# OpenRobotLab/EmbodiedScan

Hardware: NVIDIA H100
Metric: training scans/sec mv-3ddet 20-view (ResNet-50/16 + MinkResNet34, 480x640, 100k pts) (higher is better)
Workload: dtype bf16

## Files before the change

embodiedscan_b200/csrc/scratch.cu:

```cuda
#include <mutex>

#include "common.cuh"

namespace {

__global__ void sum_partial_rows_kernel(const float* __restrict__ part, int n_parts, long long width, float* __restrict__ out,
                                        int accumulate) {
  const long long j = blockIdx.x * (long long)blockDim.x + threadIdx.x;
  if (j >= width) return;
  float s = accumulate ? out[j] : 0.f;
  for (int p = 0; p < n_parts; ++p) s += part[(long long)p * width + j];
  out[j] = s;
}

}

int esb_sm_count() {
  static int sms[64] = {};
  int dev = 0;
  cudaGetDevice(&dev);
  if (dev >= 64) return 132;
  if (sms[dev] == 0) {
    int n = 132;
    cudaDeviceGetAttribute(&n, cudaDevAttrMultiProcessorCount, dev);
    sms[dev] = n;
  }
  return sms[dev];
}

namespace {
constexpr unsigned long long kScratchKeepBytes = 512ull << 20;
std::mutex g_pool_mutex;
cudaMemPool_t g_pool[64] = {};

cudaMemPool_t scratch_pool(int dev, cudaStream_t s) {
  if (dev < 0 || dev >= 64) return nullptr;
  std::lock_guard<std::mutex> lock(g_pool_mutex);
  if (g_pool[dev] == nullptr) {
    cudaStreamCaptureStatus st = cudaStreamCaptureStatusNone;
    cudaStreamIsCapturing(s, &st);
    if (st != cudaStreamCaptureStatusNone) return nullptr;
    cudaMemPoolProps props = {};
    props.allocType = cudaMemAllocationTypePinned;
    props.location.type = cudaMemLocationTypeDevice;
    props.location.id = dev;
    cudaMemPool_t pool = nullptr;
    if (cudaMemPoolCreate(&pool, &props) != cudaSuccess) return nullptr;
    unsigned long long keep = kScratchKeepBytes;
    cudaMemPoolSetAttribute(pool, cudaMemPoolAttrReleaseThreshold, &keep);
    g_pool[dev] = pool;
  }
  return g_pool[dev];
}
}

cudaError_t esb_scratch_alloc(void** p, size_t bytes, cudaStream_t s) {
  int dev = 0;
  cudaGetDevice(&dev);
  const size_t n = bytes > 0 ? bytes : 16;
  cudaMemPool_t pool = scratch_pool(dev, s);
  return pool != nullptr ? cudaMallocFromPoolAsync(p, n, pool, s) : cudaMallocAsync(p, n, s);
}

cudaError_t esb_scratch_free(void* p, cudaStream_t s) { return cudaFreeAsync(p, s); }

int esb_sum_partial_rows(const float* part, int n_parts, long long width, float* out, int accumulate, cudaStream_t s) {
  if (width == 0) return ESB_OK;
  sum_partial_rows_kernel<<<esb_div_up(width, 256), 256, 0, s>>>(part, n_parts, width, out, accumulate);
  ESB_CUDA_LAUNCH_CHECK("sum_partial_rows_kernel");
  return ESB_OK;
}
```

embodiedscan_b200/csrc/spconv_tc.cu:

```cuda
#include "tc_common.cuh"

using namespace esb_tc;

namespace {

__global__ void tile_mask_kernel(const int* __restrict__ nbr, int K, int n, uint32_t* __restrict__ masks) {
  const int tile = blockIdx.x, r = threadIdx.x;
  const int row = tile * TC_M + r;
  uint32_t m = 0;
  if (row < n)
    for (int k = 0; k < K; ++k)
      if (nbr[(long long)k * n + row] >= 0) m |= 1u << k;
  m = __reduce_or_sync(0xffffffffu, m);
  __shared__ uint32_t s[4];
  if ((r & 31) == 0) s[r >> 5] = m;
  __syncthreads();
  if (r == 0) masks[tile] = s[0] | s[1] | s[2] | s[3];
}

template <int N_TILE, int STAGES, bool B_MN>
__global__ void __launch_bounds__(384, 1)
spconv_tc_fwd_kernel(const __nv_bfloat16* __restrict__ x, const __grid_constant__ CUtensorMap tmw,
                     const int* __restrict__ nbr, const uint32_t* __restrict__ masks, __nv_bfloat16* __restrict__ y,
                     int n_out, int cin, int cout, int K) {
  constexpr int A_BYTES = A_STAGE_BYTES;
  constexpr int B_STAGE_BYTES = N_TILE * 128;
  constexpr int STAGE_BYTES = A_BYTES + B_STAGE_BYTES;
  constexpr int LAG = STAGES - 2;
  constexpr int NPROD = 128;
  constexpr int NCONS = 256;
  constexpr int PITCH = N_TILE + 4;
  static_assert(TC_M * PITCH * 4 <= STAGES * STAGE_BYTES, "the accumulator image reuses the stage buffers");
  extern __shared__ __align__(1024) uint8_t smem_raw[];
  uint8_t* smem = (uint8_t*)(((uintptr_t)smem_raw + 1023) & ~(uintptr_t)1023);
  uint64_t* full_bar = (uint64_t*)(smem + STAGES * STAGE_BYTES);
  uint64_t* empty_bar = full_bar + STAGES;
  uint64_t* accum_bar = empty_bar + STAGES;
  float* img = reinterpret_cast<float*>(smem);
  __shared__ int idx_s[2][NPROD];

  const int tile = blockIdx.x;
  const int n0 = blockIdx.y * N_TILE;
  const uint32_t mask = masks[tile];
  const int nchunk = cin / TC_BK;
  const int total = __popc(mask) * nchunk;

  if (threadIdx.x == 0) {
    for (int s = 0; s < STAGES; ++s) {
      mbar_init(&full_bar[s], NPROD + 1);
      mbar_init(&empty_bar[s], NCONS / 32);
    }
    mbar_init(accum_bar, NCONS);
    asm volatile("fence.mbarrier_init.release.cluster;" ::: "memory");
    tma_prefetch_desc(&tmw);
  }
  __syncthreads();

  if (threadIdx.x >= NCONS) {
    const int t = threadIdx.x - NCONS;
    const int sub = t & 7, rgrp = t >> 3;
    const uint32_t sw = (uint32_t)(rgrp & 7);
    const uint32_t a_thread_off = (uint32_t)((rgrp >> 3) * 1024 + (rgrp & 7) * 128) + ((sub ^ sw) << 4);
    int it = 0, kcount = 0;
    const int my_row = tile * TC_M + t;
    int v_next = (mask && my_row < n_out) ? nbr[(long long)(__ffs(mask) - 1) * n_out + my_row] : -1;
    for (uint32_t mk = mask; mk; mk &= mk - 1, ++kcount) {
      const int k = __ffs(mk) - 1;
      int* idx_buf = idx_s[kcount & 1];
      idx_buf[t] = v_next;
      asm volatile("bar.sync 1, %0;" ::"n"(NPROD) : "memory");
      {
        const uint32_t rest = mk & (mk - 1);
        v_next = (rest && my_row < n_out) ? nbr[(long long)(__ffs(rest) - 1) * n_out + my_row] : -1;
      }
      int src[8];
#pragma unroll
      for (int i = 0; i < 8; ++i) src[i] = idx_buf[rgrp + 16 * i];
      for (int c = 0; c < nchunk; ++c, ++it) {
        const int s = it % STAGES;
        if (it >= STAGES) mbar_wait(&empty_bar[s], ((it / STAGES) - 1) & 1);
        const uint32_t stage_base = smem_u32(smem + s * STAGE_BYTES);
        if (t == 0) {
          mbar_expect_tx(&full_bar[s], B_STAGE_BYTES);
          const uint32_t b_base = stage_base + A_BYTES;
          if (B_MN) {
#pragma unroll
            for (int a = 0; a < N_TILE / 64; ++a) tma_load_2d(&tmw, &full_bar[s], b_base + a * 8192, n0 + a * 64, k * cin + c * TC_BK);
          } else {
            tma_load_2d(&tmw, &full_bar[s], b_base, c * TC_BK, k * cout + n0);
          }
        }
        const uint32_t a_base = stage_base + a_thread_off;
#pragma unroll
        for (int i = 0; i < 8; ++i)
          cp_async16_ca(a_base + i * 2048, x + (long long)(src[i] >= 0 ? src[i] : 0) * cin + c * TC_BK + sub * 8,
                        src[i] >= 0 ? 16 : 0);
        cp_async_commit();
        if (it >= LAG) {
          cp_async_wait<LAG>();
          fence_proxy_async();
          mbar_arrive(&full_bar[(it - LAG) % STAGES]);
        }
      }
    }
    cp_async_wait<0>();
    fence_proxy_async();
    for (int d = (total > LAG ? total - LAG : 0); d < total; ++d) mbar_arrive(&full_bar[d % STAGES]);

    const int row = tile * TC_M + t;
    if (total > 0) mbar_wait(accum_bar, 0);
    __nv_bfloat16* yrow = y + (long long)row * cout + n0;
#pragma unroll 1
    for (int c0 = 0; c0 < N_TILE; c0 += 32) {
      uint32_t v[32];
      if (total > 0) {
        img_ld<32>(img, PITCH, t, c0, v);
      } else {
#pragma unroll
        for (int i = 0; i < 32; ++i) v[i] = 0u;
      }
      if (row < n_out) {
#pragma unroll
        for (int q = 0; q < 4; ++q) {
          uint4 o;
          o.x = pack_bf16(v[8 * q + 0], v[8 * q + 1]);
          o.y = pack_bf16(v[8 * q + 2], v[8 * q + 3]);
          o.z = pack_bf16(v[8 * q + 4], v[8 * q + 5]);
          o.w = pack_bf16(v[8 * q + 6], v[8 * q + 7]);
          *reinterpret_cast<uint4*>(yrow + c0 + 8 * q) = o;
        }
      }
    }
  } else if (total > 0) {
    const int wg = threadIdx.x >> 7;
    float acc[N_TILE / 2];
    for (int it = 0; it < total; ++it) {
      const int s = it % STAGES;
      mbar_wait(&full_bar[s], (it / STAGES) & 1);
      const uint32_t a_addr = smem_u32(smem + s * STAGE_BYTES) + wg * 8192;
      const uint32_t b_addr = smem_u32(smem + s * STAGE_BYTES) + A_BYTES;
      wgmma_fence();
#pragma unroll
      for (int kk = 0; kk < TC_BK / 16; ++kk) {
        const uint64_t bd = B_MN ? make_desc(b_addr + kk * 2048, 8192, 1024) : make_desc(b_addr + kk * 32, 16, 1024);
        wgmma_bf16<N_TILE, 0, B_MN ? 1 : 0>(acc, make_desc(a_addr + kk * 32, 16, 1024), bd, it > 0 || kk > 0);
      }
      wgmma_commit();
      wgmma_wait<1>();
      if (it > 0 && (threadIdx.x & 31) == 0) mbar_arrive(&empty_bar[(it - 1) % STAGES]);
    }
    wgmma_wait<0>();
    acc_fence<N_TILE / 2>(acc);
    asm volatile("bar.sync 2, %0;" ::"n"(NCONS) : "memory");
    acc_store<N_TILE>(acc, img, PITCH, wg * 64, threadIdx.x & 127);
    mbar_arrive(accum_bar);
  }
}

template <int N_TILE, int STAGES>
__global__ void __launch_bounds__(384, 1)
spconv_tc_wgrad_kernel(const __nv_bfloat16* __restrict__ x, const __nv_bfloat16* __restrict__ dy,
                       const int* __restrict__ pair_in, const int* __restrict__ pair_out,
                       const int* __restrict__ k_offsets, float* __restrict__ part, int cin, int cout, int K,
                       int chunk_pairs) {
  constexpr int A_BYTES = 64 * 256;
  constexpr int B_BYTES = 64 * N_TILE * 2;
  constexpr int STAGE_BYTES = A_BYTES + B_BYTES;
  constexpr int LAG = STAGES - 2;
  constexpr int NCONS = 256;
  constexpr int PITCH = N_TILE + 4;
  static_assert(128 * PITCH * 4 <= STAGES * STAGE_BYTES, "the accumulator image reuses the stage buffers");
  extern __shared__ __align__(1024) uint8_t smem_raw[];
  uint8_t* smem = (uint8_t*)(((uintptr_t)smem_raw + 1023) & ~(uintptr_t)1023);
  uint64_t* full_bar = (uint64_t*)(smem + STAGES * STAGE_BYTES);
  uint64_t* empty_bar = full_bar + STAGES;
  uint64_t* accum_bar = empty_bar + STAGES;

  int k = 0, chunk = blockIdx.x, p_beg = 0, p_end = 0;
  for (; k < K; ++k) {
    p_beg = k_offsets[k];
    p_end = k_offsets[k + 1];
    const int nch = (p_end - p_beg + chunk_pairs - 1) / chunk_pairs;
    if (chunk < nch) break;
    chunk -= nch;
  }
  if (k >= K) return;
  const int ci0 = blockIdx.y * 128, co0 = blockIdx.z * N_TILE;
  const int s_beg = p_beg + chunk * chunk_pairs;
  const int s_end = min(p_end, s_beg + chunk_pairs);
  const int total = (s_end - s_beg + 63) / 64;

  if (threadIdx.x == 0) {
    for (int s = 0; s < STAGES; ++s) {
      mbar_init(&full_bar[s], 128);
      mbar_init(&empty_bar[s], NCONS / 32);
    }
    mbar_init(accum_bar, NCONS);
    asm volatile("fence.mbarrier_init.release.cluster;" ::: "memory");
  }
  __syncthreads();
  const int a_ch = min(128, cin - ci0);

  if (threadIdx.x >= NCONS) {
    const int t = threadIdx.x - NCONS;
    const int warp = t >> 5;
    const int mc = t & 15, kk0 = t >> 4;
    const bool a_ok_ch = mc * 8 < a_ch;
    int ri[8], ro[8];
#pragma unroll
    for (int q = 0; q < 8; ++q) {
      const int p = s_beg + kk0 + 8 * q;
      ri[q] = p < s_end ? pair_in[p] : -1;
      ro[q] = p < s_end ? pair_out[p] : -1;
    }
    for (int it = 0; it < total; ++it) {
      const int s = it % STAGES;
      if (it >= STAGES) mbar_wait(&empty_bar[s], ((it / STAGES) - 1) & 1);
      const uint32_t a_base = smem_u32(smem + s * STAGE_BYTES);
      const uint32_t b_base = a_base + A_BYTES;
#pragma unroll
      for (int q = 0; q < 8; ++q) {
        const int kk = kk0 + 8 * q;
        const bool ok = ri[q] >= 0 && a_ok_ch;
        const uint32_t dst = a_base + (mc >> 3) * 8192 + (kk >> 3) * 1024 + (kk & 7) * 128 + (((mc & 7) ^ (kk & 7)) << 4);
        cp_async16_cg(dst, x + (long long)(ok ? ri[q] : 0) * cin + ci0 + mc * 8, ok ? 16 : 0);
      }
#pragma unroll
      for (int q = 0; q < N_TILE / 16; ++q) {
        const int idx = q * 128 + t;
        const int kk = idx / (N_TILE / 8), nc = idx % (N_TILE / 8);
        int rr;
        if (N_TILE == 128) {
          rr = ro[q];
        } else {
          const int p = s_beg + it * 64 + kk;
          rr = p < s_end ? pair_out[p] : -1;
        }
        const uint32_t dst = b_base + (nc >> 3) * 8192 + (kk >> 3) * 1024 + (kk & 7) * 128 + (((nc & 7) ^ (kk & 7)) << 4);
        cp_async16_cg(dst, dy + (long long)(rr >= 0 ? rr : 0) * cout + co0 + nc * 8, rr >= 0 ? 16 : 0);
      }
      cp_async_commit();
      if (it + 1 < total) {
#pragma unroll
        for (int q = 0; q < 8; ++q) {
          const int p = s_beg + (it + 1) * 64 + kk0 + 8 * q;
          ri[q] = p < s_end ? pair_in[p] : -1;
          ro[q] = p < s_end ? pair_out[p] : -1;
        }
      }
      if (it >= LAG) {
        cp_async_wait<LAG>();
        fence_proxy_async();
        mbar_arrive(&full_bar[(it - LAG) % STAGES]);
      }
    }
    cp_async_wait<0>();
    fence_proxy_async();
    for (int d = (total > LAG ? total - LAG : 0); d < total; ++d) mbar_arrive(&full_bar[d % STAGES]);

    mbar_wait(accum_bar, 0);
    const float* stg = reinterpret_cast<const float*>(smem);
    const int lane = t & 31;
    for (int rr = 0; rr < 32; ++rr) {
      const int r = warp * 32 + rr;
      const int ci = ci0 + r;
      if (ci >= cin) break;
      float* dwrow = part + ((long long)blockIdx.x * cin + ci) * cout + co0;
#pragma unroll
      for (int c = lane * 4; c < N_TILE; c += 128)
        *reinterpret_cast<float4*>(dwrow + c) = *reinterpret_cast<const float4*>(stg + r * PITCH + c);
    }
  } else {
    const int wg = threadIdx.x >> 7;
    float acc[N_TILE / 2];
    for (int it = 0; it < total; ++it) {
      const int s = it % STAGES;
      mbar_wait(&full_bar[s], (it / STAGES) & 1);
      const uint32_t a_addr = smem_u32(smem + s * STAGE_BYTES) + wg * 8192;
      const uint32_t b_addr = smem_u32(smem + s * STAGE_BYTES) + A_BYTES;
      wgmma_fence();
#pragma unroll
      for (int kk = 0; kk < 4; ++kk)
        wgmma_bf16<N_TILE, 1, 1>(acc, make_desc(a_addr + kk * 2048, 8192, 1024), make_desc(b_addr + kk * 2048, 8192, 1024), it > 0 || kk > 0);
      wgmma_commit();
      wgmma_wait<1>();
      if (it > 0 && (threadIdx.x & 31) == 0) mbar_arrive(&empty_bar[(it - 1) % STAGES]);
    }
    wgmma_wait<0>();
    acc_fence<N_TILE / 2>(acc);
    asm volatile("bar.sync 2, %0;" ::"n"(NCONS) : "memory");
    acc_store<N_TILE>(acc, reinterpret_cast<float*>(smem), PITCH, wg * 64, threadIdx.x & 127);
    mbar_arrive(accum_bar);
  }
}

__global__ void spconv_wgrad_reduce_kernel(const float* __restrict__ part, const int* __restrict__ k_offsets, float* __restrict__ dw,
                                           int cin, int cout, int K, int chunk_pairs) {
  const long long e = blockIdx.x * (long long)blockDim.x + threadIdx.x;
  const long long per_k = (long long)cin * cout;
  if (e >= per_k * K) return;
  const int k = (int)(e / per_k);
  const long long j = e - k * per_k;
  int c0 = 0;
  for (int kk = 0; kk < k; ++kk) c0 += (k_offsets[kk + 1] - k_offsets[kk] + chunk_pairs - 1) / chunk_pairs;
  const int nch = (k_offsets[k + 1] - k_offsets[k] + chunk_pairs - 1) / chunk_pairs;
  float s = dw[e];
  for (int c = c0; c < c0 + nch; ++c) s += part[(long long)c * per_k + j];
  dw[e] = s;
}

template <int N_TILE, int STAGES, bool B_MN>
int launch_fwd(const void* x, const CUtensorMap& tmw, const int* nbr, const unsigned* masks, void* y, long long n_out, int cin,
               int cout, int K, cudaStream_t stream) {
  size_t smem = (size_t)STAGES * (A_STAGE_BYTES + N_TILE * 128) + 1024 + 256;
  auto kern = spconv_tc_fwd_kernel<N_TILE, STAGES, B_MN>;
  cudaError_t e = cudaFuncSetAttribute(kern, cudaFuncAttributeMaxDynamicSharedMemorySize, (int)smem);
  if (e != cudaSuccess) { esb_set_error("spconv_tc_fwd: smem attr: %s", cudaGetErrorString(e)); return ESB_ECUDA; }
  dim3 grid(esb_div_up(n_out, TC_M), cout / N_TILE);
  kern<<<grid, 384, smem, stream>>>((const __nv_bfloat16*)x, tmw, nbr, masks, (__nv_bfloat16*)y, (int)n_out, cin,
                                              cout, K);
  return ESB_OK;
}

template <int N_TILE, int STAGES>
int launch_wgrad(const void* x, const void* dy, const int* pin, const int* pout, const int* koff, float* part, int cin,
                 int cout, int K, int n_chunks, int chunk_pairs, cudaStream_t stream) {
  size_t smem = (size_t)STAGES * (64 * 256 + 64 * N_TILE * 2) + 1024 + 256;
  auto kern = spconv_tc_wgrad_kernel<N_TILE, STAGES>;
  cudaError_t e = cudaFuncSetAttribute(kern, cudaFuncAttributeMaxDynamicSharedMemorySize, (int)smem);
  if (e != cudaSuccess) { esb_set_error("spconv_tc_wgrad: smem attr: %s", cudaGetErrorString(e)); return ESB_ECUDA; }
  dim3 grid(n_chunks, esb_div_up(cin, 128), cout / N_TILE);
  kern<<<grid, 384, smem, stream>>>((const __nv_bfloat16*)x, (const __nv_bfloat16*)dy, pin, pout, koff, part, cin, cout, K,
                                    chunk_pairs);
  return ESB_OK;
}

}

extern "C" int esb_kmap_tile_masks(const int* nbr, int K, long long n, unsigned* masks, void* stream) {
  ESB_CHECK_ARG(K >= 1 && K <= 32, "esb_kmap_tile_masks: K must be in [1,32]");
  if (n == 0) return ESB_OK;
  tile_mask_kernel<<<esb_div_up(n, TC_M), 128, 0, (cudaStream_t)stream>>>(nbr, K, (int)n, masks);
  ESB_CUDA_LAUNCH_CHECK("tile_mask_kernel");
  return ESB_OK;
}

extern "C" int esb_spconv_tc_fwd(const void* x, const void* wt, const int* nbr, const unsigned* masks, void* y,
                                 long long n_out, int cin, int cout, int K, int w_layout, void* stream_) {
  cudaStream_t stream = (cudaStream_t)stream_;
  ESB_CHECK_ARG(cin % 64 == 0 && cout % 64 == 0 && cin > 0 && cout > 0, "esb_spconv_tc_fwd: channels must be multiples of 64");
  ESB_CHECK_ARG(K >= 1 && K <= 27, "esb_spconv_tc_fwd: K must be in [1,27]");
  if (n_out == 0) return ESB_OK;
  int rc;
  const int sms = esb_sm_count();
  long long row_tiles = (n_out + TC_M - 1) / TC_M;
  const int n_tile = (cout % 256 == 0 && row_tiles * (cout / 256) >= sms) ? 256
                     : (cout % 128 == 0 && row_tiles * (cout / 128) >= sms) ? 128 : 64;
  CUtensorMap tmw;
  {
    unsigned long long dims[2], str[1];
    unsigned box[2];
    if (w_layout) {
      dims[0] = (unsigned long long)cout; dims[1] = (unsigned long long)K * cin; str[0] = (unsigned long long)cout * 2;
      box[0] = 64; box[1] = 64;
    } else {
      dims[0] = (unsigned long long)cin; dims[1] = (unsigned long long)K * cout; str[0] = (unsigned long long)cin * 2;
      box[0] = 64; box[1] = (unsigned)n_tile;
    }
    rc = esb_tma_encode(&tmw, wt, 2, dims, str, box, nullptr, 128);
    if (rc != ESB_OK) return rc;
  }
#define ESB_TC_LAUNCH(NT, ST)                                                                       \
  (w_layout ? launch_fwd<NT, ST, true>(x, tmw, nbr, masks, y, n_out, cin, cout, K, stream)         \
            : launch_fwd<NT, ST, false>(x, tmw, nbr, masks, y, n_out, cin, cout, K, stream))
  if (n_tile == 256)
    rc = ESB_TC_LAUNCH(256, 4);
  else if (n_tile == 128)
    rc = ESB_TC_LAUNCH(128, 4);
  else
    rc = ESB_TC_LAUNCH(64, 4);
#undef ESB_TC_LAUNCH
  if (rc != ESB_OK) return rc;
  ESB_CUDA_LAUNCH_CHECK("spconv_tc_fwd_kernel");
  return ESB_OK;
}

extern "C" int esb_spconv_tc_wgrad(const void* x, const void* dy, const int* pair_in, const int* pair_out,
                                   const int* k_offsets, float* dw, long long n_pairs_hint, int cin, int cout, int K,
                                   void* stream_) {
  cudaStream_t stream = (cudaStream_t)stream_;
  ESB_CHECK_ARG(cin % 64 == 0 && cout % 64 == 0 && cin > 0 && cout > 0, "esb_spconv_tc_wgrad: channels must be multiples of 64");
  int n_tile = (cout % 128 == 0) ? 128 : 64;
  long long tiles = (long long)esb_div_up(cin, 128) * (cout / n_tile);
  long long target_chunks = (4LL * 2 * esb_sm_count() + tiles - 1) / tiles;
  long long cp = (n_pairs_hint / 2 + target_chunks - 1) / target_chunks;
  cp = (cp + 63) / 64 * 64;
  if (cp < 512) cp = 512;
  if (cp > 16384) cp = 16384;
  int chunk_pairs = (int)cp;
  int n_chunks = (int)(n_pairs_hint / chunk_pairs) + K + 1;
  float* part = nullptr;
  ESB_CUDA_CALL(esb_scratch_alloc((void**)&part, sizeof(float) * n_chunks * cin * cout, stream));
  int rc = n_tile == 128
               ? launch_wgrad<128, 3>(x, dy, pair_in, pair_out, k_offsets, part, cin, cout, K, n_chunks, chunk_pairs, stream)
               : launch_wgrad<64, 4>(x, dy, pair_in, pair_out, k_offsets, part, cin, cout, K, n_chunks, chunk_pairs, stream);
  if (rc == ESB_OK) {
    spconv_wgrad_reduce_kernel<<<esb_div_up((long long)K * cin * cout, 256), 256, 0, stream>>>(part, k_offsets, dw, cin, cout, K,
                                                                                             chunk_pairs);
  }
  ESB_CUDA_CALL(esb_scratch_free(part, stream));
  if (rc != ESB_OK) return rc;
  ESB_CUDA_LAUNCH_CHECK("spconv_tc_wgrad_kernel");
  return ESB_OK;
}
```

Baseline: 49.99.

## Parallelize partial-row sums across rows and vectorize spconv wgrad split-K reduction

The generic partial-row summation kernel now lets several threads of a block load different partial rows of the same column, stage them through shared memory, and have one thread per column add them in the original order, so narrow-width reductions are no longer stuck with one serial thread per column. Column width per block is chosen adaptively from the width and the SM count. The spconv weight-gradient reduce kernel now processes four outputs per thread with float4 loads and batches eight chunk loads ahead to hide latency. Summation order is kept sequential for determinism, but the code assumes cin*cout is a multiple of 4 and adds shared-memory and sync overhead.

```diff
diff --git a/embodiedscan_b200/csrc/scratch.cu b/embodiedscan_b200/csrc/scratch.cu
--- a/embodiedscan_b200/csrc/scratch.cu
+++ b/embodiedscan_b200/csrc/scratch.cu
@@ -4,13 +4,87 @@
 
 namespace {
 
-__global__ void sum_partial_rows_kernel(const float* __restrict__ part, int n_parts, long long width, float* __restrict__ out,
-                                        int accumulate) {
-  const long long j = blockIdx.x * (long long)blockDim.x + threadIdx.x;
-  if (j >= width) return;
-  float s = accumulate ? out[j] : 0.f;
-  for (int p = 0; p < n_parts; ++p) s += part[(long long)p * width + j];
-  out[j] = s;
+constexpr int kSumThreads = 256;
+constexpr int kSumLoads = 8;
+constexpr int kSumTile = kSumThreads * kSumLoads;
+
+__device__ __forceinline__ float add_chain_contiguous(const float* __restrict__ tile, int n, float s) {
+  const float4* q = reinterpret_cast<const float4*>(tile);
+  float4 a[4];
+#pragma unroll
+  for (int u = 0; u < 4; ++u) a[u] = q[u];
+  int r = 0;
+  for (; r + 16 <= n; r += 16) {
+    const int nx = min(r + 16, kSumTile - 16) / 4;
+    float4 b[4];
+#pragma unroll
+    for (int u = 0; u < 4; ++u) b[u] = q[nx + u];
+#pragma unroll
+    for (int u = 0; u < 4; ++u) {
+      s = __fadd_rn(s, a[u].x);
+      s = __fadd_rn(s, a[u].y);
+      s = __fadd_rn(s, a[u].z);
+      s = __fadd_rn(s, a[u].w);
+    }
+#pragma unroll
+    for (int u = 0; u < 4; ++u) a[u] = b[u];
+  }
+  const float rest[16] = {a[0].x, a[0].y, a[0].z, a[0].w, a[1].x, a[1].y, a[1].z, a[1].w,
+                          a[2].x, a[2].y, a[2].z, a[2].w, a[3].x, a[3].y, a[3].z, a[3].w};
+#pragma unroll
+  for (int u = 0; u < 16; ++u)
+    if (r + u < n) s = __fadd_rn(s, rest[u]);
+  return s;
+}
+
+__global__ void __launch_bounds__(kSumThreads) sum_partial_rows_kernel(const float* __restrict__ part, int n_parts,
+                                                                       long long width, float* __restrict__ out,
+                                                                       int accumulate, int cw) {
+  __shared__ __align__(16) float tile[kSumTile];
+  const int t = threadIdx.x;
+  const int rows = kSumTile / cw, rstep = kSumThreads / cw;
+  const int r0 = t / cw;
+  const long long j = blockIdx.x * (long long)cw + (t & (cw - 1));
+  const bool col_ok = j < width;
+  const bool adder = t < cw && col_ok;
+  float v[kSumLoads];
+  auto load = [&](int p0) {
+#pragma unroll
+    for (int k = 0; k < kSumLoads; ++k) {
+      const int p = p0 + r0 + k * rstep;
+      v[k] = col_ok && p < n_parts ? part[(long long)p * width + j] : 0.f;
+    }
+  };
+  float s = adder && accumulate ? out[j] : 0.f;
+  if (n_parts > 0) load(0);
+  for (int p0 = 0; p0 < n_parts; p0 += rows) {
+    __syncthreads();
+#pragma unroll
+    for (int k = 0; k < kSumLoads; ++k) tile[t + k * kSumThreads] = v[k];
+    __syncthreads();
+    if (p0 + rows < n_parts) load(p0 + rows);
+    if (adder && cw == 1) {
+      s = add_chain_contiguous(tile, min(rows, n_parts - p0), s);
+    } else if (adder) {
+      const int n = min(rows, n_parts - p0);
+      const float* col = tile + t;
+      float a[16];
+#pragma unroll
+      for (int u = 0; u < 16; ++u) a[u] = col[min(u, n - 1) * cw];
+      int r = 0;
+      for (; r + 16 <= n; r += 16) {
+        float b[16];
+#pragma unroll
+        for (int u = 0; u < 16; ++u) b[u] = col[min(r + 16 + u, n - 1) * cw];
+#pragma unroll
+        for (int u = 0; u < 16; ++u) s = __fadd_rn(s, a[u]);
+#pragma unroll
+        for (int u = 0; u < 16; ++u) a[u] = b[u];
+      }
+      for (int u = 0; r + u < n; ++u) s = __fadd_rn(s, col[(r + u) * cw]);
+    }
+  }
+  if (adder) out[j] = s;
 }
 
 }
@@ -66,7 +140,10 @@
 
 int esb_sum_partial_rows(const float* part, int n_parts, long long width, float* out, int accumulate, cudaStream_t s) {
   if (width == 0) return ESB_OK;
-  sum_partial_rows_kernel<<<esb_div_up(width, 256), 256, 0, s>>>(part, n_parts, width, out, accumulate);
+  int cw = 1;
+  while (cw < 8 && cw < width) cw *= 2;
+  while (cw < kSumThreads && (width + cw - 1) / cw > 8LL * esb_sm_count()) cw *= 2;
+  sum_partial_rows_kernel<<<esb_div_up(width, cw), kSumThreads, 0, s>>>(part, n_parts, width, out, accumulate, cw);
   ESB_CUDA_LAUNCH_CHECK("sum_partial_rows_kernel");
   return ESB_OK;
 }
diff --git a/embodiedscan_b200/csrc/spconv_tc.cu b/embodiedscan_b200/csrc/spconv_tc.cu
--- a/embodiedscan_b200/csrc/spconv_tc.cu
+++ b/embodiedscan_b200/csrc/spconv_tc.cu
@@ -296,7 +296,8 @@
 
 __global__ void spconv_wgrad_reduce_kernel(const float* __restrict__ part, const int* __restrict__ k_offsets, float* __restrict__ dw,
                                            int cin, int cout, int K, int chunk_pairs) {
-  const long long e = blockIdx.x * (long long)blockDim.x + threadIdx.x;
+  constexpr int D = 8;
+  const long long e = (blockIdx.x * (long long)blockDim.x + threadIdx.x) * 4;
   const long long per_k = (long long)cin * cout;
   if (e >= per_k * K) return;
   const int k = (int)(e / per_k);
@@ -304,9 +305,25 @@
   int c0 = 0;
   for (int kk = 0; kk < k; ++kk) c0 += (k_offsets[kk + 1] - k_offsets[kk] + chunk_pairs - 1) / chunk_pairs;
   const int nch = (k_offsets[k + 1] - k_offsets[k] + chunk_pairs - 1) / chunk_pairs;
-  float s = dw[e];
-  for (int c = c0; c < c0 + nch; ++c) s += part[(long long)c * per_k + j];
-  dw[e] = s;
+  float s[4] = {dw[e], dw[e + 1], dw[e + 2], dw[e + 3]};
+  const float4* src = reinterpret_cast<const float4*>(part + (long long)c0 * per_k + j);
+  const long long stride = per_k / 4;
+  for (int c = 0; c < nch; c += D) {
+    float4 v[D];
+#pragma unroll
+    for (int u = 0; u < D; ++u)
+      if (c + u < nch) v[u] = src[(c + u) * stride];
+#pragma unroll
+    for (int u = 0; u < D; ++u)
+      if (c + u < nch) {
+        s[0] = __fadd_rn(s[0], v[u].x);
+        s[1] = __fadd_rn(s[1], v[u].y);
+        s[2] = __fadd_rn(s[2], v[u].z);
+        s[3] = __fadd_rn(s[3], v[u].w);
+      }
+  }
+#pragma unroll
+  for (int q = 0; q < 4; ++q) dw[e + q] = s[q];
 }
 
 template <int N_TILE, int STAGES, bool B_MN>
@@ -405,8 +422,8 @@
                ? launch_wgrad<128, 3>(x, dy, pair_in, pair_out, k_offsets, part, cin, cout, K, n_chunks, chunk_pairs, stream)
                : launch_wgrad<64, 4>(x, dy, pair_in, pair_out, k_offsets, part, cin, cout, K, n_chunks, chunk_pairs, stream);
   if (rc == ESB_OK) {
-    spconv_wgrad_reduce_kernel<<<esb_div_up((long long)K * cin * cout, 256), 256, 0, stream>>>(part, k_offsets, dw, cin, cout, K,
-                                                                                             chunk_pairs);
+    spconv_wgrad_reduce_kernel<<<esb_div_up((long long)K * cin * cout / 4, 256), 256, 0, stream>>>(part, k_offsets, dw, cin, cout,
+                                                                                                 K, chunk_pairs);
   }
   ESB_CUDA_CALL(esb_scratch_free(part, stream));
   if (rc != ESB_OK) return rc;
```

After: 61.36, median of 6. 1.23x the previous value.
